# JohnLonginotto/uq

Hardware: AMD Instinct MI355X
Metric: FASTQ encode MB/s (150bp synthetic; bit-exact tables vs reference) (higher is better)
Workload: dtype u8

## Files before the change

uq_amd/csrc/pack.hip:

```cpp
#include "common.h"
#include "swar.h"
#include "lines.h"
#include "histo.h"

namespace {
constexpr int PK_THREADS = 256;

struct PackLut {
    int16_t dna_code[256];
    int16_t qual_code[256];
    int16_t n_qual[256];
};

struct PackGeom {
    uint32_t R;
    uint32_t Rs;
    uint32_t Cd, Cq;
    uint32_t G;
    uint32_t variable;
    uint32_t stage_bytes;
    uint32_t out_bytes;
    uint32_t magicG;
    uint32_t dna_max;
    uint32_t fill_d, fill_q;
// ... 27 lines not shown
    if constexpr ((4 * B) % 8 == 0) return i < B / 2 ? a1 >> (8 * i) : a0 >> (8 * (i - B / 2));
    else
#endif
    return (uint32_t)((((uint64_t)a0 << (4 * B)) | a1) >> (8 * i));
}

template <bool CLEAR = false>
__device__ __noinline__ void store_tile_any(uint8_t* gdst, uint8_t* lsrc, uint32_t nb, uint32_t tid) {
    const uint32_t mis = (uint32_t)(uintptr_t)gdst;
    if ((mis & 15) == 0) {
        const uint32_t nv = nb >> 4;
        for (uint32_t i = tid; i < nv; i += 256) { ((uint4*)gdst)[i] = ((const uint4*)lsrc)[i]; if (CLEAR) ((uint4*)lsrc)[i] = make_uint4(0, 0, 0, 0); }
        for (uint32_t i = (nv << 4) + tid; i < nb; i += 256) { gdst[i] = lsrc[i]; if (CLEAR) lsrc[i] = 0; }
    } else if ((mis & 7) == 0) {
        const uint32_t nv = nb >> 3;
        for (uint32_t i = tid; i < nv; i += 256) { ((uint2*)gdst)[i] = ((const uint2*)lsrc)[i]; if (CLEAR) ((uint2*)lsrc)[i] = make_uint2(0, 0); }
        for (uint32_t i = (nv << 3) + tid; i < nb; i += 256) { gdst[i] = lsrc[i]; if (CLEAR) lsrc[i] = 0; }
    } else if ((mis & 3) == 0) {
        const uint32_t nv = nb >> 2;
        for (uint32_t i = tid; i < nv; i += 256) { ((uint32_t*)gdst)[i] = ((const uint32_t*)lsrc)[i]; if (CLEAR) ((uint32_t*)lsrc)[i] = 0; }
        for (uint32_t i = (nv << 2) + tid; i < nb; i += 256) { gdst[i] = lsrc[i]; if (CLEAR) lsrc[i] = 0; }
    } else {
        for (uint32_t i = tid; i < nb; i += 256) { gdst[i] = lsrc[i]; if (CLEAR) lsrc[i] = 0; }
    }
}
template <bool CLEAR = false>
__device__ __forceinline__ void store_tile(uint8_t* gdst, uint8_t* lsrc, uint32_t nb, uint32_t tid) {
    if ((((uint32_t)(uintptr_t)gdst) & 15u) == 0 && (nb & 15u) == 0) {
#pragma unroll 1
        for (uint32_t i = tid; i < (nb >> 4); i += 256) { ((uint4*)gdst)[i] = ((const uint4*)lsrc)[i]; if (CLEAR) ((uint4*)lsrc)[i] = make_uint4(0, 0, 0, 0); }
    } else store_tile_any<CLEAR>(gdst, lsrc, nb, tid);
}

struct QnLds {
    uint8_t line1[256 + 16];
    uint8_t inset[256];
    uint8_t seps[32];
    uint32_t vmin[UQ_QF_MAXC], vmax[UQ_QF_MAXC];
    uint32_t flags, on, plen, slen, nsep, l1len;
    uint32_t sepset;
    uint32_t seps_lo, seps_hi;
    uint32_t pow10[10];
};

__device__ __forceinline__ uint32_t eq_bytes(uint32_t w, uint32_t c4) {
    const uint32_t x = w ^ c4;
    return ~((((x & 0x7F7F7F7Fu) + 0x7F7F7F7Fu) | x)) & 0x80808080u;
}
__device__ __forceinline__ uint32_t nondigit_bytes(uint32_t w) {
    const uint32_t lo7 = w & 0x7F7F7F7Fu;
    return (~(lo7 + 0x50505050u) | (lo7 + 0x46464646u) | w) & 0x80808080u;
}
__device__ __forceinline__ uint32_t low_bytes(uint32_t n) { return n >= 4 ? 0xFFFFFFFFu : ~(0xFFFFFFFFu << (8 * n)); }

__device__ __forceinline__ void lds_window12(const uint8_t* base, int32_t o, uint32_t& w0, uint32_t& w1, uint32_t& w2) {
    const uint32_t* p = (const uint32_t*)(base + (o & ~3));
    const uint32_t a = p[0], b = p[1], c = p[2], d = p[3];
    const uint32_t sh = (uint32_t)o & 3u;
    w0 = __builtin_amdgcn_alignbyte(b, a, sh);
    w1 = __builtin_amdgcn_alignbyte(c, b, sh);
    w2 = __builtin_amdgcn_alignbyte(d, c, sh);
}

__device__ __forceinline__ void qname_tile(const uint8_t* stage, const uint32_t* meta, uint32_t q, QnLds* s, uint32_t* __restrict__ vals, uint64_t pitch,
                                           uint64_t row) {
    const uint32_t qs = meta[4 * q], ql = meta[4 * q + 1] - qs - 1;
    const uint32_t plen = s->plen, slen = s->slen, nsep = s->nsep, l1len = s->l1len;
// ... 47 lines not shown
        }
        if (bad) f |= 16u;
        const unsigned long long want = (unsigned long long)s->seps_lo | ((unsigned long long)s->seps_hi << 32);
        if (found != nsep || eseq != want) f |= 1u;
        uint32_t start = plen;
        for (uint32_t c = 0; c <= nsep && c < UQ_QF_MAXC; ++c) {
            uint32_t stop = c == nsep ? end : (uint32_t)(epos >> (8 * c)) & 0xFFu;
            if (stop < start || stop > end) stop = start;
            const uint32_t nd = stop - start;
            uint32_t w0, w1, w2;
            lds_window12(stage, (int32_t)(qs + stop) - 12, w0, w1, w2);
            const uint32_t keep = nd > 9 ? 9u : nd;
            const uint32_t k2 = low_bytes(keep >= 4 ? 0u : 4u - keep), k1 = keep <= 4 ? 0xFFFFFFFFu : (keep >= 8 ? 0u : low_bytes(8u - keep)),
                           k0 = keep <= 8 ? 0xFFFFFFFFu : low_bytes(12u - keep);
            const uint32_t d0 = w0 & 0x0F0F0F0Fu & ~k0, d1 = w1 & 0x0F0F0F0Fu & ~k1, d2 = w2 & 0x0F0F0F0Fu & ~k2;
            uint32_t mag = d0 >> 24;
            mag = mag * 10 + (d1 & 0xFFu); mag = mag * 10 + ((d1 >> 8) & 0xFFu); mag = mag * 10 + ((d1 >> 16) & 0xFFu); mag = mag * 10 + (d1 >> 24);
            mag = mag * 10 + (d2 & 0xFFu); mag = mag * 10 + ((d2 >> 8) & 0xFFu); mag = mag * 10 + ((d2 >> 16) & 0xFFu); mag = mag * 10 + (d2 >> 24);
            if (nd > 9) f |= 4u;
            else if (nd == 0 || (nd > 1 && mag < s->pow10[nd - 1])) f |= 16u;
            vals[c * pitch + row] = mag;
            if (mag < s->vmin[c]) atomicMin(&s->vmin[c], mag);
            if (mag > s->vmax[c]) atomicMax(&s->vmax[c], mag);
            start = stop + 1;
        }
        if (ql < l1len && !differs && !(f & 32u)) f |= 128u;
        if (ql < l1len && s->line1[l1len - ql] == s->line1[0]) f |= 128u;
    }
    if (f) atomicOr(&s->flags, f);
}

constexpr int PK_NV = 5;
constexpr int PK_NV_STATS = 4;
#ifdef PK_ONE_COPY
constexpr int pks_copies(int bd, bool four_wg) { return bd == 3 ? 4 : 1; }
#else
constexpr int pks_copies(int bd, bool four_wg) { return bd == 2 && four_wg ? 8 : 4; }
#endif
constexpr uint32_t pks_bins(int bd) { return bd == 3 ? 512u : 256u; }
constexpr uint32_t pks_words(int bd, bool four_wg) { return pks_bins(bd) * pks_copies(bd, four_wg) + 128; }

struct TileRec { uint64_t start; uint32_t T, A, B, pad; };
struct PackLists {
    CensusView cv;
    const uint32_t* over;
};

__global__ __launch_bounds__(256) void tile_origin_kernel(CensusView cv, const unsigned long long* __restrict__ d_async, const uint32_t* __restrict__ over, uint64_t first,
                                                          uint64_t n, uint64_t R, uint64_t entries, TileRec* __restrict__ rec, unsigned long long* __restrict__ bad) {
    const uint64_t tt = (uint64_t)blockIdx.x * 256 + threadIdx.x;
    if (tt == 0) *bad = UQ_NONE;
    if (tt >= entries) return;
    uint64_t nlines = 4 * (first + n);
    if (d_async) {
        nlines = d_async[0];
        const uint64_t have = nlines / 4;
        if (have < n) n = have;
        if (d_async[1] || *over) n = 0;
    }
    uint64_t r = tt * R;
    if (r > n) r = n;
    uint32_t T, kk;
    cv_locate(cv, (int64_t)(4 * (first + r)) - 1, T, kk);
    bool ok;
    TileRec out;
    out.start = n ? cv_line_start(cv, nlines, T, kk, 0, ok) : 0;
    uint32_t c[3];
#pragma unroll
    for (uint32_t k = 0; k < 3; ++k) {
        const uint64_t t = (uint64_t)T + k;
        c[k] = t < cv.nb ? (uint32_t)((t + 1 < cv.nb ? (uint64_t)cv.offs[t + 1] : nlines) - cv.offs[t]) : 0u;
        if (c[k] > CV_LIST_CAP) c[k] = CV_LIST_CAP;
    }
    out.T = T; out.A = kk | (c[0] << 16); out.B = c[1] | (c[2] << 16); out.pad = 0;
    rec[tt] = out;
}

template <int BD, int BQ, bool NTRICK, bool FAST, bool STATS, bool QN, bool LISTS = false, bool VAR = false>
__global__ __launch_bounds__(PK_THREADS, (STATS && (NTRICK || QN)) ? 4 : 5) void pack_tile_kernel(const uint8_t* __restrict__ buf,
                                                               const uint64_t* __restrict__ ls, uint64_t first,
                                                               uint64_t n, PackLut lut, PackGeom g,
                                                               uint8_t* __restrict__ dna, uint8_t* __restrict__ qual,
                                                               unsigned long long* __restrict__ bad,
                                                               uq_stats* __restrict__ st, const unsigned long long* __restrict__ d_async,
                                                               uq_qname_fused* __restrict__ qf, uint32_t* __restrict__ qvals, uint64_t qpitch, PackLists pl,
                                                               const TileRec* __restrict__ trec) {
    constexpr int NV = STATS ? PK_NV_STATS : PK_NV;
    extern __shared__ __align__(16) uint8_t smem[];
    uint8_t* stage = smem + 16;
    uint8_t* out_d = stage + g.stage_bytes;
    uint32_t* meta = (uint32_t*)(out_d + g.out_bytes);
    int16_t* l_dna = (int16_t*)(meta + 4 * g.R + 4);
    int16_t* l_qual = l_dna + 256;
    int16_t* l_nq = l_qual + 256;

    const uint32_t tid = threadIdx.x;
    l_dna[tid] = lut.dna_code[tid];
    l_qual[tid] = lut.qual_code[tid];
    if (NTRICK) l_nq[tid] = lut.n_qual[tid];
    RecordAcc acc;
    bool incomplete = false;
    constexpr bool FOUR_WG = STATS && (NTRICK || QN);
    constexpr int PKS_COPIES = pks_copies(BD, FOUR_WG);
    __shared__ uint32_t cnt_tab[STATS ? pks_words(BD, FOUR_WG) : 1];
    uint32_t fill_pairs = 0, n_pairs = 0;
    constexpr uint32_t PKS_BINS = pks_bins(BD), PKS_WORDS = pks_words(BD, FOUR_WG);
    if (STATS) for (uint32_t i = tid; i < PKS_WORDS; i += PK_THREADS) cnt_tab[i] = 0;
    if (VAR) for (uint32_t i = tid; i < (g.out_bytes >> 4); i += PK_THREADS) ((uint4*)out_d)[i] = make_uint4(0, 0, 0, 0);
    QnLds* qn = (QnLds*)(l_nq + 256);
    bool qn_on = false;
    if (STATS && QN) qn_on = qf->ok != 0;
    if (STATS && QN) {
        qn->line1[tid] = qf->line1[tid]; qn->inset[tid] = qf->inset[tid];
        if (tid < 16) qn->line1[256 + tid] = 0;
        if (tid < 32) qn->seps[tid] = qf->seps[tid];
        if (tid < UQ_QF_MAXC) { qn->vmin[tid] = 0xFFFFFFFFu; qn->vmax[tid] = 0; }
        if (tid == 0) {
            qn->flags = 0; qn->plen = qf->plen; qn->slen = qf->slen; qn->nsep = qf->nsep; qn->l1len = qf->l1len;
            uint32_t set = 0x01010101u * qf->seps[0], nset = 1, lo = 0, hi = 0;
            for (uint32_t k = 0; k < qf->nsep && k < 8; ++k) {
                const uint32_t c = qf->seps[k];
                if (k < 4) lo |= c << (8 * k); else hi |= c << (8 * (k - 4));
                bool seen = false;
                for (uint32_t m = 0; m < nset; ++m) seen = seen || ((set >> (8 * m)) & 0xFFu) == c;
                if (!seen && nset < 4) { set = (set & ~(0xFFu << (8 * nset))) | (c << (8 * nset)); ++nset; }
            }
            qn->sepset = set; qn->seps_lo = lo; qn->seps_hi = hi;
            uint32_t pw = 1;
            for (uint32_t k = 0; k < 10; ++k) { qn->pow10[k] = pw; pw *= 10; }
        }
    }
    uint64_t nl_total = 4 * (first + n);
    constexpr bool lists = STATS && LISTS;
    if (d_async) {
        nl_total = d_async[0];
        const uint64_t have = d_async[0] / 4;
        if (have > n) incomplete = true; else n = have;
        if (d_async[1] || (lists && *pl.over)) { incomplete = true; n = 0; }
    }

    const uint64_t R = g.R;
    const uint64_t ntiles = (n + R - 1) / R;
    const uint64_t S = gridDim.x;
    struct Bounds { uint64_t g0, g1; uint32_t pT, pA, pB; };
    struct Regs { uint4 v[NV]; uint64_t m0; uint64_t g0; uint32_t skew, nvec, Rt, mrel, mraw; bool ok; };
    struct RawBounds { uint32_t lo, hi; };
    auto load_raw = [&](uint64_t tt) {
        RawBounds x{0u, 0u};
        if (tt < ntiles) {
            const uint32_t ln = lane_id();
            if constexpr (lists) {
                x.lo = ((const uint32_t*)(trec + tt))[ln < 8u ? ln : 0u];
            } else {
                const uint32_t Rn = (uint32_t)((n - tt * R) < R ? (n - tt * R) : R);
                const uint64_t v = ls[4 * (first + tt * R) + (ln == 1u ? 4 * Rn : 0u)];
                x.lo = (uint32_t)v; x.hi = (uint32_t)(v >> 32);
            }
        }
        return x;
    };
    auto bounds_of = [&](uint64_t tt, const RawBounds& x) {
        auto lane = [](uint32_t v, int k) { return (uint32_t)__builtin_amdgcn_readlane((int)v, k); };
        Bounds b{0, 0, 0, 0, 0};
        if (tt < ntiles) {
            if constexpr (lists) {
                b.g0 = (uint64_t)lane(x.lo, 0) | ((uint64_t)lane(x.lo, 1) << 32);
                b.pT = lane(x.lo, 2); b.pA = lane(x.lo, 3); b.pB = lane(x.lo, 4);
                b.g1 = (uint64_t)lane(x.lo, 6) | ((uint64_t)lane(x.lo, 7) << 32);
            } else {
                b.g0 = (uint64_t)lane(x.lo, 0) | ((uint64_t)lane(x.hi, 0) << 32);
                b.g1 = (uint64_t)lane(x.lo, 1) | ((uint64_t)lane(x.hi, 1) << 32);
            }
        }
        return b;
    };
    auto load_bounds = [&](uint64_t tt) {
        Bounds b{0, 0, 0, 0, 0};
        if (tt < ntiles) {
            const uint32_t Rn = (uint32_t)((n - tt * R) < R ? (n - tt * R) : R);
            if constexpr (lists) {
                const TileRec r0 = trec[tt];
                b.g0 = r0.start; b.pT = r0.T; b.pA = r0.A; b.pB = r0.B; b.g1 = trec[tt + 1].start;
            }
            else { b.g0 = ls[4 * (first + tt * R)]; b.g1 = ls[4 * (first + tt * R) + 4 * Rn]; }
        }
        return b;
    };
    auto tile_reads = [&](uint64_t tt) -> uint32_t { return tt < ntiles ? (uint32_t)((n - tt * R) < R ? (n - tt * R) : R) : 0u; };
    auto issue = [&](uint64_t rfirst, uint32_t cnt, Bounds b) {
        Regs x;
        x.ok = false; x.m0 = 0; x.g0 = b.g0; x.skew = 0; x.nvec = 0; x.Rt = 0; x.mrel = 0; x.mraw = 0;
#pragma unroll
        for (int u = 0; u < NV; ++u) x.v[u] = make_uint4(0, 0, 0, 0);
        if (cnt == 0) return x;
        x.Rt = cnt;
        const uint64_t a0 = ((uint64_t)(uintptr_t)buf + b.g0) & ~uint64_t(15);
        x.skew = (uint32_t)(((uint64_t)(uintptr_t)buf + b.g0) - a0);
        const uint64_t span = b.g1 - b.g0 + x.skew;
        x.nvec = (uint32_t)((span + 15) >> 4);
        x.ok = span + 32 <= g.stage_bytes && x.nvec <= (uint32_t)(NV * PK_THREADS);
        if constexpr (lists) {
            const uint32_t kk = b.pA & 0xFFFFu, avail = (b.pA >> 16) + (b.pB & 0xFFFFu) + (b.pB >> 16);
            if (kk + 4 * cnt > avail) x.ok = false;
        }
        if (!x.ok) return x;
        const uint4* src = (const uint4*)(buf + ((int64_t)b.g0 - (int64_t)x.skew));
#pragma unroll
        for (int u = 0; u < NV; ++u) { const uint32_t i = u * PK_THREADS + tid; if (i < x.nvec) x.v[u] = src[i]; }
        if (tid <= 4 * x.Rt) {
            if constexpr (lists) {
                uint32_t idx = (b.pA & 0xFFFFu) + tid, t = b.pT;
                const uint32_t c0 = b.pA >> 16, c1 = b.pB & 0xFFFFu;
                if (idx > c0) { idx -= c0; ++t; if (idx > c1) { idx -= c1; ++t; } }
                x.mrel = x.skew - (uint32_t)b.g0 + (idx == 0 ? 0u : (uint32_t)t * (uint32_t)CV_TILE - pl.cv.mis + 1u);
                x.mraw = idx == 0 ? 0u : (uint32_t)pl.cv.list[(uint64_t)t * CV_LIST_CAP + (idx - 1)];
            } else x.m0 = ls[4 * (first + rfirst) + tid];
        }
        return x;
    };

    uint32_t rr, pp;
    fast_divmod(tid, g.P, g.magicP, rr, pp);
    uint32_t badr = 0xFFFFFFFFu;
    uint64_t bad_tile = UQ_NONE;
    auto do_tile = [&](const uint64_t r0, const Regs& cur, auto&& between) {
        const uint32_t Rt = cur.Rt;
        uint8_t* out_q = out_d + ((Rt * g.Cd + 15) & ~15u);
        if (cur.ok) {
            if (tid <= 4 * Rt) meta[tid] = lists ? cur.mrel + cur.mraw : (uint32_t)(cur.m0 - cur.g0) + cur.skew;
#pragma unroll
            for (int u = 0; u < NV; ++u) { const uint32_t i = u * PK_THREADS + tid; if (i < cur.nvec) ((uint4*)stage)[i] = cur.v[u]; }
        } else {
            if (tid == 0) bad_tile = bad_tile < r0 ? bad_tile : r0;
            incomplete = true;
            if (STATS && QN && qn_on && tid == 0) atomicOr(&qf->flags, 256u);
        }
        __syncthreads();
        const bool ok = cur.ok;
        between();
#ifndef PK_ABL_NOQN
        if (STATS && QN && qn_on && ok && tid >= PK_THREADS - 64 && tid - (PK_THREADS - 64) < Rt)
            qname_tile(stage, meta, tid - (PK_THREADS - 64), qn, qvals, qpitch, r0 + (tid - (PK_THREADS - 64)));
#endif
        if (ok) {
            auto pack_group = [&](const uint32_t r, const uint32_t L, const int32_t wd, const uint32_t shd, const int32_t wq, const uint32_t shq, uint8_t* orow_d,
                                  uint8_t* orow_q, const uint32_t gg) {
                const int32_t j0 = (int32_t)L - 8 * (int32_t)gg - 8;
                uint32_t ad0 = 0, ad1 = 0, aq0 = 0, aq1 = 0;
                if (j0 > -8) {
                uint32_t b_lo, b_hi, q_lo, q_hi;
                lds_window8_at(stage, wd, shd, b_lo, b_hi);
                lds_window8_at(stage, wq, shq, q_lo, q_hi);
                if (j0 < 0) {
                    uint32_t mlo, mhi;
                    window_masks((uint32_t)(-j0), mlo, mhi);
                    b_lo = bfi(mlo, b_lo, g.fill_d); b_hi = bfi(mhi, b_hi, g.fill_d);
                    q_lo = bfi(mlo, q_lo, g.fill_q); q_hi = bfi(mhi, q_hi, g.fill_q);
                }
                bool generic = !FAST;
                if (FAST) {
                    uint32_t c0, c1, e0, e1;
                    if constexpr (BD == 2) {
                        c0 = acgt_codes(b_lo); c1 = acgt_codes(b_hi);
                        e0 = acgt_chars(c0) ^ b_lo; e1 = acgt_chars(c1) ^ b_hi;
                    } else {
                        c0 = __builtin_amdgcn_perm(g.i2c_hi, g.i2c_lo, (b_lo >> g.h_shift) & 0x07070707u);
                        c1 = __builtin_amdgcn_perm(g.i2c_hi, g.i2c_lo, (b_hi >> g.h_shift) & 0x07070707u);
                        e0 = __builtin_amdgcn_perm(g.c2c_hi, g.c2c_lo, c0) ^ b_lo; e1 = __builtin_amdgcn_perm(g.c2c_hi, g.c2c_lo, c1) ^ b_hi;
                    }
                    uint32_t u0 = q_lo + g.q_addlo, u1 = q_hi + g.q_addlo;
                    uint32_t bq0 = (q_lo | (q_lo + g.q_addhi) | ~u0) & 0x80808080u;
                    uint32_t bq1 = (q_hi | (q_hi + g.q_addhi) | ~u1) & 0x80808080u;
                    uint32_t x0 = u0 & 0x7F7F7F7Fu, x1 = u1 & 0x7F7F7F7Fu;
                    if (e0 | e1) {
                        if (NTRICK && !((q_lo | q_hi) & 0x80808080u)) {
// ... 34 lines not shown
                                    atomicAdd((uint32_t*)(hb + b0 * (4 * PKS_COPIES)), 1u);
                                    atomicAdd((uint32_t*)(hb + b1 * (4 * PKS_COPIES)), 1u);
                                }
                            }
                            if (j0 < 0) fill_pairs += (uint32_t)(-j0);
                            if (NTRICK && (e0 | e1)) {
                                const uint32_t m0 = nonzero_bytes(e0), m1 = nonzero_bytes(e1);
                                const uint32_t ne0 = nonzero_bytes(q_lo ^ g.n_qchar), ne1 = nonzero_bytes(q_hi ^ g.n_qchar);
                                n_pairs += (uint32_t)__popc(m0 & 0x01010101u) + (uint32_t)__popc(m1 & 0x01010101u);
                                if ((m0 & ne0) | (m1 & ne1)) incomplete = true;
                            }
                        }
                    }
                }
                if (generic) {
                    const uint32_t cbw[2] = {b_lo, b_hi};
                    const uint32_t cqw[2] = {q_lo, q_hi};
                    uint32_t ad[2] = {0, 0}, aq[2] = {0, 0};
                    int32_t orall = 0;
#pragma unroll
                    for (int k = 0; k < 8; ++k) {
                        const uint32_t cb = (cbw[k >> 2] >> (8 * (k & 3))) & 255u;
                        const uint32_t cc = (cqw[k >> 2] >> (8 * (k & 3))) & 255u;
                        int32_t dc = l_dna[cb];
                        int32_t qc = l_qual[cc];
                        if (NTRICK) {
                            if (dc < 0) { dc = 0; qc = l_nq[cb]; }
                        }
                        orall |= dc | qc;
                        ad[k >> 2] = (ad[k >> 2] << BD) | (uint32_t)dc;
                        aq[k >> 2] = (aq[k >> 2] << BQ) | (uint32_t)qc;
                    }
                    if (orall < 0) {
                        badr = badr < (uint32_t)(r0 + r) ? badr : (uint32_t)(r0 + r);
                        ad[0] = ad[1] = aq[0] = aq[1] = 0;
                    }
                    ad0 = ad[0]; ad1 = ad[1]; aq0 = aq[0]; aq1 = aq[1];
                }
                }
                if (g.variable) {
                    const int32_t i = (int32_t)L - 8 * (int32_t)gg;
                    if (i >= 0 && i < 4) { ad1 |= 1u << (BD * i); aq1 |= 1u << (BQ * i); }
                    else if (i >= 4 && i < 8) { ad0 |= 1u << (BD * (i - 4)); aq0 |= 1u << (BQ * (i - 4)); }
                }
                uint8_t* od = orow_d - BD * gg;
                uint8_t* oq = orow_q - BQ * gg;
#ifdef PK_ABL_NOSTORE
                if ((ad0 ^ aq0) == 0x12345678u && (ad1 ^ aq1) == 0x9ABCDEF0u) od[0] = 1;
                else if (false)
#endif
                if (gg + 1 < g.G) {
#pragma unroll
                    for (int i = 0; i < BD; ++i) od[-i] = (uint8_t)group_byte<BD>(ad0, ad1, i);
#pragma unroll
                    for (int i = 0; i < BQ; ++i) oq[-i] = (uint8_t)group_byte<BQ>(aq0, aq1, i);
                } else {
                    const uint32_t nd = g.Cd - BD * gg, nq = g.Cq - BQ * gg;
#pragma unroll
                    for (int i = 0; i < BD; ++i)
                        if ((uint32_t)i < nd) od[-i] = (uint8_t)group_byte<BD>(ad0, ad1, i);
#pragma unroll
                    for (int i = 0; i < BQ; ++i)
                        if ((uint32_t)i < nq) oq[-i] = (uint8_t)group_byte<BQ>(aq0, aq1, i);
                }
            };
            if (rr < Rt) {
                const uint32_t r = rr;
                const uint32_t so = meta[4 * r + 1];
                uint32_t L = meta[4 * r + 2] - so - 1;
                const uint32_t qo = meta[4 * r + 3];
                if (STATS) {
                    const uint32_t Lq = meta[4 * r + 4] - qo - 1;
#ifndef PK_ABL_NOREC
                    if (pp == 0) acc.record(r0 + r, stage[meta[4 * r + 2]] == '+', L, Lq, meta[4 * r + 4] - meta[4 * r]);
#endif
                    if (L > g.dna_max || Lq != L) incomplete = true;
                }
                if (L > g.dna_max || meta[4 * r + 4] - qo - 1 != L) { badr = badr < (uint32_t)(r0 + r) ? badr : (uint32_t)(r0 + r); L = 0; }
                uint8_t* orow_d = out_d + r * g.Cd + (g.Cd - 1);
                uint8_t* orow_q = out_q + r * g.Cq + (g.Cq - 1);
                const uint32_t gend = VAR ? (((L + 8) >> 3) < g.G ? ((L + 8) >> 3) : g.G) : g.G;
#ifndef PK_ABL_NOGROUP
                int32_t wd = (int32_t)(so + L) - 8 * (int32_t)pp - 8, wq = (int32_t)(qo + L) - 8 * (int32_t)pp - 8;
                const uint32_t shd = (uint32_t)wd & 3u, shq = (uint32_t)wq & 3u;
                wd &= ~3; wq &= ~3;
                const int32_t wstep = 8 * (int32_t)g.P;
                for (uint32_t gg = pp; gg < gend; gg += g.P, wd -= wstep, wq -= wstep) pack_group(r, L, wd, shd, wq, shq, orow_d, orow_q, gg);
#endif
            }
        }
        __syncthreads();
#ifndef PK_NO_EARLY_WAIT
        __builtin_amdgcn_s_waitcnt(0x0F70);
#endif
        if (ok) {
            if constexpr (STATS && (NTRICK || QN)) {
                store_tile<VAR>(dna + r0 * g.Cd, out_d, Rt * g.Cd, tid);
                store_tile<VAR>(qual + r0 * g.Cq, out_q, Rt * g.Cq, tid);
            } else {
                store_tile_any<VAR>(dna + r0 * g.Cd, out_d, Rt * g.Cd, tid);
                store_tile_any<VAR>(qual + r0 * g.Cq, out_q, Rt * g.Cq, tid);
            }
        }
    };

    uint64_t t = blockIdx.x;
    constexpr bool VBOUNDS = STATS && (NTRICK || QN);
    using NextBounds = std::conditional_t<VBOUNDS, RawBounds, Bounds>;
    auto fetch_next = [&](uint64_t tt) -> NextBounds { if constexpr (VBOUNDS) return load_raw(tt); else return load_bounds(tt); };
    auto next_bounds = [&](uint64_t tt, const NextBounds& x) -> Bounds { if constexpr (VBOUNDS) return bounds_of(tt, x); else return x; };
    NextBounds b_next = fetch_next(t + S);
    Regs cur = issue(t * R, tile_reads(t), load_bounds(t));
#ifndef PK_NO_EARLY_WAIT
    __builtin_amdgcn_s_waitcnt(0x0F70);
#endif
    for (; t < ntiles; t += S) {
        NextBounds b_nn{};
        if constexpr (!VBOUNDS) b_nn = fetch_next(t + 2 * S);
        if (cur.ok) {
            const Regs now = cur;
            do_tile(t * R, now, [&] {
                cur = issue((t + S) * R, tile_reads(t + S), next_bounds(t + S, b_next));
                if constexpr (VBOUNDS) b_next = fetch_next(t + 2 * S); else b_next = b_nn;
            });
        } else {
            const uint32_t Rt = cur.Rt;
            for (uint32_t sub = 0; sub < Rt; sub += g.Rs) {
                const uint32_t cnt = Rt - sub < g.Rs ? Rt - sub : g.Rs;
                const uint64_t rf = t * R + sub;
                Bounds sb{0, 0, 0, 0, 0};
                if constexpr (lists) {
                    uint32_t T, kk; bool found;
                    cv_locate(pl.cv, (int64_t)(4 * (first + rf)) - 1, T, kk);
                    sb.g0 = cv_line_start(pl.cv, nl_total, T, kk, 0, found); sb.g1 = cv_line_start(pl.cv, nl_total, T, kk, 4 * cnt, found);
                    uint32_t c[3];
#pragma unroll
                    for (uint32_t k = 0; k < 3; ++k) {
                        const uint64_t tq = (uint64_t)T + k;
                        c[k] = tq < pl.cv.nb ? (uint32_t)((tq + 1 < pl.cv.nb ? (uint64_t)pl.cv.offs[tq + 1] : nl_total) - pl.cv.offs[tq]) : 0u;
                        if (c[k] > CV_LIST_CAP) c[k] = CV_LIST_CAP;
                    }
                    sb.pT = T; sb.pA = kk | (c[0] << 16); sb.pB = c[1] | (c[2] << 16);
                } else { sb.g0 = ls[4 * (first + rf)]; sb.g1 = ls[4 * (first + rf) + 4 * cnt]; }
                const Regs piece = issue(rf, cnt, sb);
                do_tile(rf, piece, [] {});
                __syncthreads();
            }
            cur = issue((t + S) * R, tile_reads(t + S), next_bounds(t + S, b_next));
            if constexpr (VBOUNDS) b_next = fetch_next(t + 2 * S); else b_next = b_nn;
#ifndef PK_NO_EARLY_WAIT
            __builtin_amdgcn_s_waitcnt(0x0F70);
#endif
        }
    }
    if (badr != 0xFFFFFFFFu) atomicMin(bad, (unsigned long long)badr);
    if (bad_tile != UQ_NONE) atomicMin(bad, (unsigned long long)bad_tile);
    if (STATS) {
        if (fill_pairs) atomicSub(&cnt_tab[lane_id() & (PKS_COPIES - 1)], fill_pairs);
        if (NTRICK && n_pairs) {
            atomicSub(&cnt_tab[((g.n_code & 0xFFu) * PKS_COPIES) + (lane_id() & (PKS_COPIES - 1))], n_pairs);
            atomicAdd(&cnt_tab[PKS_BINS * PKS_COPIES], n_pairs);
        }
        __syncthreads();
        const uint32_t qmin = 0x80u - (g.q_addlo & 0xFFu);
        for (uint32_t bin = tid; bin < PKS_BINS; bin += PK_THREADS) {
            uint32_t v = 0;
#pragma unroll
            for (int c = 0; c < PKS_COPIES; ++c) v += cnt_tab[bin * PKS_COPIES + c];
            const uint32_t code = bin >> 6;
            const uint32_t base = BD == 2 ? (0x54474341u >> (8 * code)) & 0xFFu
                                          : ((code < 4 ? g.c2c_lo >> (8 * code) : g.c2c_hi >> (8 * (code - 4))) & 0xFFu);
            if (v) atomicAdd((unsigned long long*)&st->counts[base * 256 + qmin + (bin & 63u)], (unsigned long long)v);
        }
        if (NTRICK && tid == 0) {
            const uint32_t v = cnt_tab[PKS_BINS * PKS_COPIES];
            if (v) atomicAdd((unsigned long long*)&st->counts[(g.n_char & 0xFFu) * 256 + (g.n_qchar & 0xFFu)], (unsigned long long)v);
        }
        acc.flush(st, first);
        if (incomplete) st->reserved = 1;
        if (QN) {
            if (qn_on && tid < UQ_QF_MAXC && qn->vmin[tid] <= qn->vmax[tid]) { atomicMin(&qf->vmin[tid], qn->vmin[tid]); atomicMax(&qf->vmax[tid], qn->vmax[tid]); }
            if (qn_on && tid == 0 && qn->flags) atomicOr(&qf->flags, qn->flags);
            if (blockIdx.x == 0 && tid == 0) qf->nreads = n;
        }
    }
}

__global__ __launch_bounds__(256) void pack_carry_kernel(const uint8_t* __restrict__ buf, const uint64_t* __restrict__ ls,
                                                         uint64_t first, uint64_t n, PackLut lut, uint32_t bd, uint32_t bq,
                                                         uint32_t Cd, uint32_t Cq, uint32_t variable,
                                                         uint8_t* __restrict__ dna, uint8_t* __restrict__ qual,
                                                         unsigned long long* __restrict__ bad) {
    __shared__ int16_t l_dna[256], l_qual[256], l_nq[256];
    l_dna[threadIdx.x] = lut.dna_code[threadIdx.x];
    l_qual[threadIdx.x] = lut.qual_code[threadIdx.x];
    l_nq[threadIdx.x] = lut.n_qual[threadIdx.x];
    __syncthreads();
    const uint64_t r = (uint64_t)blockIdx.x * blockDim.x + threadIdx.x;
    if (r >= n) return;
    const uint64_t* p = ls + 4 * (first + r);
    const uint64_t s = p[1], q = p[3];
    const uint32_t L = (uint32_t)(p[2] - s - 1);
    uint8_t* drow = dna + r * Cd;
    uint8_t* qrow = qual + r * Cq;
    uint32_t td = 0, tq = 0, bdn = 0, bqn = 0;
    int32_t pd = (int32_t)Cd - 1, pq = (int32_t)Cq - 1;
    for (uint32_t t = 0; t < L; ++t) {
        uint32_t cb = buf[s + L - 1 - t], cc = buf[q + L - 1 - t];
        int dc = l_dna[cb], qc = l_qual[cc];
        if (dc < 0) { dc = 0; qc = l_nq[cb]; }
        if (qc < 0) { atomicMin(bad, (unsigned long long)r); qc = 0; }
        td += (uint32_t)dc << bdn; tq += (uint32_t)qc << bqn;
        bdn += bd; bqn += bq;
        while (bdn > 8) { bdn -= 8; if (pd >= 0) drow[pd] = (uint8_t)td; td >>= 8; --pd; }
        while (bqn > 8) { bqn -= 8; if (pq >= 0) qrow[pq] = (uint8_t)tq; tq >>= 8; --pq; }
    }
// ... 21 lines not shown
    if (var && lists) {
        if (qn) return bd == 3 ? pick_stats_kernel_q<3, true, true, true>(bq, ntrick) : pick_stats_kernel_q<2, true, true, true>(bq, ntrick);
        return bd == 3 ? pick_stats_kernel_q<3, false, true, true>(bq, ntrick) : pick_stats_kernel_q<2, false, true, true>(bq, ntrick);
    }
    if (qn && lists) return bd == 3 ? pick_stats_kernel_q<3, true, true>(bq, ntrick) : pick_stats_kernel_q<2, true, true>(bq, ntrick);
    if (lists) return bd == 3 ? pick_stats_kernel_q<3, false, true>(bq, ntrick) : pick_stats_kernel_q<2, false, true>(bq, ntrick);
    if (bd == 3) return qn ? pick_stats_kernel_q<3, true>(bq, ntrick) : pick_stats_kernel_q<3, false>(bq, ntrick);
    return qn ? pick_stats_kernel_q<2, true>(bq, ntrick) : pick_stats_kernel_q<2, false>(bq, ntrick);
}

template <int BD>
PackKernel pick_bq(int bq, bool ntrick, bool fast) {
    switch (bq) {
        case 1: return pick_nt<BD, 1>(ntrick, fast); case 2: return pick_nt<BD, 2>(ntrick, fast); case 3: return pick_nt<BD, 3>(ntrick, fast);
        case 4: return pick_nt<BD, 4>(ntrick, fast); case 5: return pick_nt<BD, 5>(ntrick, fast); case 6: return pick_nt<BD, 6>(ntrick, fast);
        case 7: return pick_nt<BD, 7>(ntrick, fast); default: return pick_nt<BD, 8>(ntrick, fast);
    }
}

PackKernel pick_kernel(int bd, int bq, bool ntrick, bool fast) {
    switch (bd) {
        case 1: return pick_bq<1>(bq, ntrick, fast); case 2: return pick_bq<2>(bq, ntrick, fast); case 3: return pick_bq<3>(bq, ntrick, fast);
        case 4: return pick_bq<4>(bq, ntrick, fast); case 5: return pick_bq<5>(bq, ntrick, fast); case 6: return pick_bq<6>(bq, ntrick, fast);
        case 7: return pick_bq<7>(bq, ntrick, fast); default: return pick_bq<8>(bq, ntrick, fast);
    }
}
}

static int pack_impl(uq_ctx* ctx, const uint8_t* d_buf, const uint64_t* d_line_start, uint64_t first_read,
                     uint64_t nreads, const uq_pack_params* hp, uint8_t* d_dna, uint8_t* d_qual, uint64_t* d_bad,
                     uq_stats* d_stats, int* h_fused, const unsigned long long* d_async = nullptr, uq_qname_fused* d_q = nullptr,
                     uint32_t* d_vals = nullptr, uint64_t vals_pitch = 0) {
    const bool use_lists = d_line_start == nullptr && d_async != nullptr && d_stats != nullptr;
    UQ_REQUIRE(ctx && d_buf && (d_line_start || use_lists) && hp && d_dna && d_qual && d_bad, "uq_pack: null argument");
    UQ_REQUIRE(!use_lists || (ctx->async_buf == d_buf && ctx->async_nbytes > 0), "uq_pack_stats_async: no line index given and no census of this buffer queued in front");
    if (h_fused) *h_fused = 0;
    ctx->pk_stats = ctx->pk_q = nullptr;
    if (d_stats && ctx->stats_sent == (const void*)d_stats) ctx->stats_sent = nullptr;
    UQ_REQUIRE(hp->bits_per_base >= 1 && hp->bits_per_base <= 8 && hp->bits_per_quality >= 1 && hp->bits_per_quality <= 8,
               "uq_pack: bits per symbol must be 1..8");
    const uint32_t bd = hp->bits_per_base, bq = hp->bits_per_quality;
    const uint32_t Cd = hp->dna_bytes_per_row, Cq = hp->quality_bytes_per_row;
    const uint32_t Lv = hp->dna_max + (hp->variable ? 1 : 0);
    UQ_REQUIRE(Cd == (bd * Lv + 7) / 8 && Cq == (bq * Lv + 7) / 8,
               "uq_pack: row bytes (%u, %u) do not match ceil(bits * (dna_max + variable) / 8)", Cd, Cq);
    struct BadGuard {
        uint64_t* p; hipStream_t s; bool armed;
        ~BadGuard() { if (armed) (void)hipMemsetAsync(p, 0xFF, 8, s); }
    } bad_guard{d_bad, ctx->stream, use_lists && nreads != 0};
    if (!bad_guard.armed) UQ_CHECK_HIP(hipMemsetAsync(d_bad, 0xFF, 8, ctx->stream));
    if (nreads == 0) return 0;

    PackLut lut;
    int max_d = 0, max_q = 0;
    bool ntrick = false;
    int fill_d = -1, fill_q = -1;
    for (int i = 0; i < 256; ++i) {
        lut.dna_code[i] = hp->dna_code[i];
        lut.qual_code[i] = hp->qual_code[i];
        lut.n_qual[i] = (int16_t)(hp->n_qual[i] > 32767 ? 32767 : hp->n_qual[i]);
        if (hp->dna_code[i] > max_d) max_d = hp->dna_code[i];
        if (hp->qual_code[i] > max_q) max_q = hp->qual_code[i];
        if (hp->dna_code[i] < 0 && hp->n_qual[i] >= 0) { ntrick = true; if (hp->n_qual[i] > max_q) max_q = hp->n_qual[i]; }
        if (hp->dna_code[i] == 0 && fill_d < 0) fill_d = i;
        if (hp->qual_code[i] == 0 && fill_q < 0) fill_q = i;
    }
// ... 11 lines not shown
                                                           hp->variable ? 1u : 0u, d_dna, d_qual, (unsigned long long*)d_bad);
        UQ_LAUNCH_CHECK();
        return 0;
    }

    PackGeom g;
    g.Cd = Cd; g.Cq = Cq; g.variable = hp->variable ? 1 : 0;
    g.G = (Lv + 7) / 8;
    g.dna_max = (uint32_t)hp->dna_max;
    g.magicG = magic_u32(g.G);
    g.fill_d = 0x01010101u * (uint32_t)fill_d;
    g.fill_q = 0x01010101u * (uint32_t)fill_q;
    uint32_t Rs = (stage_cap - 64) / rec;
    if (Rs > (PK_THREADS - 1) / 4) Rs = (PK_THREADS - 1) / 4;
    if (Rs == 0) Rs = 1;
    uint32_t R = Rs;
    const uint32_t avg = (uint32_t)hp->avg_record_bytes;
    if (avg >= 4 && avg < rec) {
        R = (stage_cap - 64) / (avg + avg * 15 / 100 + 1);
        if (R > (PK_THREADS - 1) / 4) R = (PK_THREADS - 1) / 4;
        if (R < Rs) R = Rs;
    }
    {
        const uint32_t out_cap = stage_cap * 3 / 4, fit = out_cap / (Cd + Cq);
        if (R > fit) R = fit > Rs ? fit : Rs;
    }
    if (R >= 4) {
        const uint32_t r16 = R & ~15u, r8 = R & ~7u, r4 = R & ~3u;
        if (r16 * 100 >= R * 85) R = r16; else if (r8 * 100 >= R * 85) R = r8; else R = r4;
    }
    if (R == 0) R = 1;
    if (Rs > R) Rs = R;
    g.R = R; g.Rs = Rs;
    g.stage_bytes = stage_cap + 32;
    g.out_bytes = (((R * Cd + 15) & ~15u) + R * Cq + 15) & ~15u;
    uint32_t P = (d_q ? PK_THREADS - 64 : PK_THREADS) / R;
    if (P > g.G) P = g.G;
    if (P < 1) P = 1;
    g.P = P; g.magicP = magic_u32(P);
    bool fast = bd == 2 && hp->dna_code['A'] == 0 && hp->dna_code['C'] == 1 && hp->dna_code['G'] == 2 && hp->dna_code['T'] == 3;
    int nbases = 0, nq = 0, qmin = 256, qmaxc = -1, ntrick_bases = 0, nchar = 0;
    for (int i = 0; i < 256; ++i) {
        if (hp->dna_code[i] >= 0) ++nbases;
        if (hp->qual_code[i] >= 0) { ++nq; if (i < qmin) qmin = i; if (i > qmaxc) qmaxc = i; }
        if (hp->dna_code[i] < 0 && hp->n_qual[i] >= 0) { ++ntrick_bases; nchar = i; }
    }
    g.h_shift = g.i2c_lo = g.i2c_hi = g.c2c_lo = g.c2c_hi = 0;
    bool fast3 = false;
    if (bd == 3 && nbases >= 1 && nbases <= 8) {
        for (uint32_t sh = 0; sh <= 4 && !fast3; ++sh) {
            uint8_t i2c[8], c2c[8]; bool used[8] = {false, false, false, false, false, false, false, false};
            memset(i2c, 0, 8); memset(c2c, 0, 8);
            bool ok = true;
            for (int ch = 1; ch < 128 && ok; ++ch) {
                const int code = hp->dna_code[ch];
                if (code < 0) continue;
                const uint32_t idx = ((uint32_t)ch >> sh) & 7u;
                if (used[idx] || code > 7) ok = false;
                else { used[idx] = true; i2c[idx] = (uint8_t)code; c2c[code] = (uint8_t)ch; }
            }
            for (int ch = 128; ch < 256 && ok; ++ch) if (hp->dna_code[ch] >= 0) ok = false;
            if (ok) {
                fast3 = true; g.h_shift = sh;
                memcpy(&g.i2c_lo, i2c, 4); memcpy(&g.i2c_hi, i2c + 4, 4); memcpy(&g.c2c_lo, c2c, 4); memcpy(&g.c2c_hi, c2c + 4, 4);
            }
        }
    }
    fast = ((fast && nbases == 4) || fast3) && nq >= 1 && qmaxc - qmin + 1 == nq && qmaxc < 128 && ntrick_bases <= 1 &&
           (ntrick_bases == 0 || (hp->n_qual[nchar] < 128 && nchar < 128));
    if (fast)
        for (int i = qmin; i <= qmaxc; ++i) fast = fast && hp->qual_code[i] == i - qmin;
    g.q_addlo = g.q_addhi = g.n_char = g.n_code = g.n_qchar = 0;
    if (fast) {
        g.q_addlo = 0x01010101u * (uint32_t)(0x80 - qmin);
        g.q_addhi = 0x01010101u * (uint32_t)(0x80 - qmin - nq);
        if (ntrick_bases == 1) {
            g.n_char = 0x01010101u * (uint32_t)nchar; g.n_code = 0x01010101u * (uint32_t)hp->n_qual[nchar];
            g.n_qchar = 0x01010101u * (uint32_t)(qmin + hp->n_qual[nchar]);
        }
    }
    if (d_stats && ((ntrick_bases == 1 && hp->n_qual[nchar] >= nq) ||
                    !fast || (bd != 2 && bd != 3) || bq > 6)) {
        return 0;
    }
    const bool var_deal = d_stats && use_lists && hp->variable;
    const size_t lds_static = d_stats ? pks_words((int)bd, ntrick || d_q != nullptr) * 4 : 4;
    const size_t lds = 16 + (size_t)g.stage_bytes + g.out_bytes + (4 * R + 4) * 4 + 3 * 512 + (d_stats ? sizeof(QnLds) : 0);
    UQ_REQUIRE(lds + lds_static <= 160 * 1024, "uq_pack: tile needs %zu bytes of LDS", lds + lds_static);
    const uint64_t tiles = (nreads + R - 1) / R;
    PackKernel k = d_stats ? pick_stats_kernel((int)bd, (int)bq, ntrick, d_q != nullptr, use_lists, var_deal) : pick_kernel((int)bd, (int)bq, ntrick, fast);
    if (lds > 48 * 1024) UQ_CHECK_HIP(hipFuncSetAttribute((const void*)k, hipFuncAttributeMaxDynamicSharedMemorySize, (int)lds));
    uint32_t per_cu = (uint32_t)((160 * 1024) / (lds + lds_static));
    {
        int cached_regs = 0;
        for (int i = 0; i < ctx->kreg_n; ++i) if (ctx->kreg_key[i] == (const void*)k) cached_regs = ctx->kreg_val[i];
        if (cached_regs == 0) {
            hipFuncAttributes fa;
            UQ_CHECK_HIP(hipFuncGetAttributes(&fa, (const void*)k));
            cached_regs = fa.numRegs > 0 ? fa.numRegs : 128;
            const int slot = ctx->kreg_n < 8 ? ctx->kreg_n++ : 7;
            ctx->kreg_key[slot] = (const void*)k; ctx->kreg_val[slot] = cached_regs;
        }
        const uint32_t alloc = ((uint32_t)(cached_regs > 0 ? cached_regs : 128) + 7) & ~7u;
        uint32_t waves_per_simd = 512 / alloc; if (waves_per_simd > 8) waves_per_simd = 8; if (waves_per_simd < 1) waves_per_simd = 1;
        const uint32_t waves_per_wg = PK_THREADS / 64;
        const uint32_t by_regs = 4 * waves_per_simd / waves_per_wg;
        if (by_regs >= 1 && by_regs < per_cu) per_cu = by_regs;
    }
    if (per_cu > 6) per_cu = 6;
    if (per_cu < 1) per_cu = 1;
    const uint64_t blocks = tiles < (uint64_t)UQ_NUM_CU * per_cu ? tiles : (uint64_t)UQ_NUM_CU * per_cu;
    PackLists pl;
    memset(&pl, 0, sizeof(pl));
    const TileRec* trec = nullptr;
    if (use_lists) {
        const uint32_t mis = (uint32_t)((uintptr_t)d_buf & 15);
        pl.cv.list = ctx->idx_bitmap; pl.cv.offs = ctx->idx_partials; pl.cv.mis = mis;
        pl.cv.nb = (((ctx->async_nbytes + mis + 15) / 16) * 16 + CV_TILE - 1) / CV_TILE;
        const uint64_t entries = tiles + 1;
// ... 54 lines not shown
```

Measured before the change: 1.474 million.

## Cut scalar register pressure in pack kernel via 32-bit indices and LDS-parked args

Switches the tile and read indices in the pack kernel from 64-bit to 32-bit, capping a call at 2^31 reads, so address arithmetic needs fewer registers. In the four-workgroup stats variants, rarely used kernel arguments (pointers, first, nl_total, Rs, census nb) are parked in LDS and reloaded only where needed. LDS is also reordered so the stage size is a compile-time constant and the lookup tables and metadata come before the variable-size output buffer. The aim is to lower SGPR/VGPR pressure and spills to help occupancy. The cost is a small extra LDS footprint, an added barrier on the sub-tile path, and the new read-count limit.

```diff
diff --git a/uq_amd/csrc/pack.hip b/uq_amd/csrc/pack.hip
--- a/uq_amd/csrc/pack.hip
+++ b/uq_amd/csrc/pack.hip
@@ -83,7 +83,7 @@
     } else store_tile_any<CLEAR>(gdst, lsrc, nb, tid);
 }
 
-struct QnLds {
+struct alignas(16) QnLds {
     uint8_t line1[256 + 16];
     uint8_t inset[256];
     uint8_t seps[32];
@@ -197,6 +197,7 @@
 
 constexpr int PK_NV = 5;
 constexpr int PK_NV_STATS = 4;
+constexpr uint32_t pk_stage_bytes(bool stats) { return (uint32_t)(stats ? PK_NV_STATS : PK_NV) * PK_THREADS * 16 + 32; }
 #ifdef PK_ONE_COPY
 constexpr int pks_copies(int bd, bool four_wg) { return bd == 3 ? 4 : 1; }
 #else
@@ -206,6 +207,7 @@
 constexpr uint32_t pks_words(int bd, bool four_wg) { return pks_bins(bd) * pks_copies(bd, four_wg) + 128; }
 
 struct TileRec { uint64_t start; uint32_t T, A, B, pad; };
+struct PkParked { unsigned long long* bad; uq_stats* st; uq_qname_fused* qf; uint64_t first, nb, nl_total; uint32_t Rs, pad; };
 struct PackLists {
     CensusView cv;
     const uint32_t* over;
@@ -252,12 +254,14 @@
                                                                const TileRec* __restrict__ trec) {
     constexpr int NV = STATS ? PK_NV_STATS : PK_NV;
     extern __shared__ __align__(16) uint8_t smem[];
+    constexpr uint32_t STAGE_BYTES = pk_stage_bytes(STATS);
     uint8_t* stage = smem + 16;
-    uint8_t* out_d = stage + g.stage_bytes;
-    uint32_t* meta = (uint32_t*)(out_d + g.out_bytes);
-    int16_t* l_dna = (int16_t*)(meta + 4 * g.R + 4);
+    int16_t* l_dna = (int16_t*)(stage + STAGE_BYTES);
     int16_t* l_qual = l_dna + 256;
     int16_t* l_nq = l_qual + 256;
+    QnLds* qn = (QnLds*)(l_nq + 256);
+    uint32_t* meta = (uint32_t*)((uint8_t*)qn + (STATS ? sizeof(QnLds) : 0));
+    uint8_t* out_d = (uint8_t*)(meta + 4 * g.R + 4);
 
     const uint32_t tid = threadIdx.x;
     l_dna[tid] = lut.dna_code[tid];
@@ -272,7 +276,6 @@
     constexpr uint32_t PKS_BINS = pks_bins(BD), PKS_WORDS = pks_words(BD, FOUR_WG);
     if (STATS) for (uint32_t i = tid; i < PKS_WORDS; i += PK_THREADS) cnt_tab[i] = 0;
     if (VAR) for (uint32_t i = tid; i < (g.out_bytes >> 4); i += PK_THREADS) ((uint4*)out_d)[i] = make_uint4(0, 0, 0, 0);
-    QnLds* qn = (QnLds*)(l_nq + 256);
     bool qn_on = false;
     if (STATS && QN) qn_on = qf->ok != 0;
     if (STATS && QN) {
@@ -295,36 +298,51 @@
             for (uint32_t k = 0; k < 10; ++k) { qn->pow10[k] = pw; pw *= 10; }
         }
     }
+    uint32_t nr = (uint32_t)n;
+#if defined(__HIP_DEVICE_COMPILE__)
+    asm("" : "+s"(nr));
+#endif
     uint64_t nl_total = 4 * (first + n);
     constexpr bool lists = STATS && LISTS;
     if (d_async) {
         nl_total = d_async[0];
         const uint64_t have = d_async[0] / 4;
-        if (have > n) incomplete = true; else n = have;
-        if (d_async[1] || (lists && *pl.over)) { incomplete = true; n = 0; }
-    }
-
-    const uint64_t R = g.R;
-    const uint64_t ntiles = (n + R - 1) / R;
-    const uint64_t S = gridDim.x;
+        if (have > nr) incomplete = true; else nr = (uint32_t)have;
+        if (d_async[1] || (lists && *pl.over)) { incomplete = true; nr = 0; }
+    }
+
+    __shared__ PkParked parked;
+    if constexpr (FOUR_WG) {
+        if (tid == 0) { parked.bad = bad; parked.st = st; parked.qf = qf; parked.first = first; parked.nb = pl.cv.nb; parked.nl_total = nl_total; parked.Rs = g.Rs; }
+    }
+    auto p_bad = [&] { if constexpr (FOUR_WG) return parked.bad; else return bad; };
+    auto p_st = [&] { if constexpr (FOUR_WG) return parked.st; else return st; };
+    auto p_qf = [&] { if constexpr (FOUR_WG) return parked.qf; else return qf; };
+    auto p_first = [&] { if constexpr (FOUR_WG) return parked.first; else return first; };
+    auto p_nl_total = [&] { if constexpr (FOUR_WG) return parked.nl_total; else return nl_total; };
+    auto p_Rs = [&] { if constexpr (FOUR_WG) return parked.Rs; else return g.Rs; };
+    auto p_cv = [&] { CensusView v = pl.cv; if constexpr (FOUR_WG) v.nb = parked.nb; return v; };
+    const uint32_t R = g.R;
+    const uint32_t ntiles = (nr + R - 1) / R;
+    const uint32_t S = gridDim.x;
     struct Bounds { uint64_t g0, g1; uint32_t pT, pA, pB; };
     struct Regs { uint4 v[NV]; uint64_t m0; uint64_t g0; uint32_t skew, nvec, Rt, mrel, mraw; bool ok; };
     struct RawBounds { uint32_t lo, hi; };
-    auto load_raw = [&](uint64_t tt) {
+    auto load_raw = [&](uint32_t tt) {
         RawBounds x{0u, 0u};
         if (tt < ntiles) {
             const uint32_t ln = lane_id();
             if constexpr (lists) {
                 x.lo = ((const uint32_t*)(trec + tt))[ln < 8u ? ln : 0u];
             } else {
-                const uint32_t Rn = (uint32_t)((n - tt * R) < R ? (n - tt * R) : R);
-                const uint64_t v = ls[4 * (first + tt * R) + (ln == 1u ? 4 * Rn : 0u)];
+                const uint32_t Rn = (nr - tt * R) < R ? (nr - tt * R) : R;
+                const uint64_t v = ls[4 * (first + (uint64_t)tt * R) + (ln == 1u ? 4 * Rn : 0u)];
                 x.lo = (uint32_t)v; x.hi = (uint32_t)(v >> 32);
             }
         }
         return x;
     };
-    auto bounds_of = [&](uint64_t tt, const RawBounds& x) {
+    auto bounds_of = [&](uint32_t tt, const RawBounds& x) {
         auto lane = [](uint32_t v, int k) { return (uint32_t)__builtin_amdgcn_readlane((int)v, k); };
         Bounds b{0, 0, 0, 0, 0};
         if (tt < ntiles) {
@@ -339,20 +357,20 @@
         }
         return b;
     };
-    auto load_bounds = [&](uint64_t tt) {
+    auto load_bounds = [&](uint32_t tt) {
         Bounds b{0, 0, 0, 0, 0};
         if (tt < ntiles) {
-            const uint32_t Rn = (uint32_t)((n - tt * R) < R ? (n - tt * R) : R);
+            const uint32_t Rn = (nr - tt * R) < R ? (nr - tt * R) : R;
             if constexpr (lists) {
                 const TileRec r0 = trec[tt];
                 b.g0 = r0.start; b.pT = r0.T; b.pA = r0.A; b.pB = r0.B; b.g1 = trec[tt + 1].start;
             }
-            else { b.g0 = ls[4 * (first + tt * R)]; b.g1 = ls[4 * (first + tt * R) + 4 * Rn]; }
+            else { b.g0 = ls[4 * (first + (uint64_t)tt * R)]; b.g1 = ls[4 * (first + (uint64_t)tt * R) + 4 * Rn]; }
         }
         return b;
     };
-    auto tile_reads = [&](uint64_t tt) -> uint32_t { return tt < ntiles ? (uint32_t)((n - tt * R) < R ? (n - tt * R) : R) : 0u; };
-    auto issue = [&](uint64_t rfirst, uint32_t cnt, Bounds b) {
+    auto tile_reads = [&](uint32_t tt) -> uint32_t { return tt < ntiles ? ((nr - tt * R) < R ? (nr - tt * R) : R) : 0u; };
+    auto issue = [&](uint32_t rfirst, uint32_t cnt, Bounds b) {
         Regs x;
         x.ok = false; x.m0 = 0; x.g0 = b.g0; x.skew = 0; x.nvec = 0; x.Rt = 0; x.mrel = 0; x.mraw = 0;
 #pragma unroll
@@ -363,7 +381,7 @@
         x.skew = (uint32_t)(((uint64_t)(uintptr_t)buf + b.g0) - a0);
         const uint64_t span = b.g1 - b.g0 + x.skew;
         x.nvec = (uint32_t)((span + 15) >> 4);
-        x.ok = span + 32 <= g.stage_bytes && x.nvec <= (uint32_t)(NV * PK_THREADS);
+        x.ok = span + 32 <= STAGE_BYTES && x.nvec <= (uint32_t)(NV * PK_THREADS);
         if constexpr (lists) {
             const uint32_t kk = b.pA & 0xFFFFu, avail = (b.pA >> 16) + (b.pB & 0xFFFFu) + (b.pB >> 16);
             if (kk + 4 * cnt > avail) x.ok = false;
@@ -379,7 +397,7 @@
                 if (idx > c0) { idx -= c0; ++t; if (idx > c1) { idx -= c1; ++t; } }
                 x.mrel = x.skew - (uint32_t)b.g0 + (idx == 0 ? 0u : (uint32_t)t * (uint32_t)CV_TILE - pl.cv.mis + 1u);
                 x.mraw = idx == 0 ? 0u : (uint32_t)pl.cv.list[(uint64_t)t * CV_LIST_CAP + (idx - 1)];
-            } else x.m0 = ls[4 * (first + rfirst) + tid];
+            } else x.m0 = ls[4 * (first + (uint64_t)rfirst) + tid];
         }
         return x;
     };
@@ -387,8 +405,8 @@
     uint32_t rr, pp;
     fast_divmod(tid, g.P, g.magicP, rr, pp);
     uint32_t badr = 0xFFFFFFFFu;
-    uint64_t bad_tile = UQ_NONE;
-    auto do_tile = [&](const uint64_t r0, const Regs& cur, auto&& between) {
+    uint32_t bad_tile = 0xFFFFFFFFu;
+    auto do_tile = [&](const uint32_t r0, const Regs& cur, auto&& between) {
         const uint32_t Rt = cur.Rt;
         uint8_t* out_q = out_d + ((Rt * g.Cd + 15) & ~15u);
         if (cur.ok) {
@@ -398,14 +416,14 @@
         } else {
             if (tid == 0) bad_tile = bad_tile < r0 ? bad_tile : r0;
             incomplete = true;
-            if (STATS && QN && qn_on && tid == 0) atomicOr(&qf->flags, 256u);
+            if (STATS && QN && qn_on && tid == 0) atomicOr(&p_qf()->flags, 256u);
         }
         __syncthreads();
         const bool ok = cur.ok;
         between();
 #ifndef PK_ABL_NOQN
         if (STATS && QN && qn_on && ok && tid >= PK_THREADS - 64 && tid - (PK_THREADS - 64) < Rt)
-            qname_tile(stage, meta, tid - (PK_THREADS - 64), qn, qvals, qpitch, r0 + (tid - (PK_THREADS - 64)));
+            qname_tile(stage, meta, tid - (PK_THREADS - 64), qn, qvals, qpitch, (uint64_t)r0 + (tid - (PK_THREADS - 64)));
 #endif
         if (ok) {
             auto pack_group = [&](const uint32_t r, const uint32_t L, const int32_t wd, const uint32_t shd, const int32_t wq, const uint32_t shq, uint8_t* orow_d,
@@ -506,7 +524,7 @@
                         aq[k >> 2] = (aq[k >> 2] << BQ) | (uint32_t)qc;
                     }
                     if (orall < 0) {
-                        badr = badr < (uint32_t)(r0 + r) ? badr : (uint32_t)(r0 + r);
+                        badr = badr < r0 + r ? badr : r0 + r;
                         ad[0] = ad[1] = aq[0] = aq[1] = 0;
                     }
                     ad0 = ad[0]; ad1 = ad[1]; aq0 = aq[0]; aq1 = aq[1];
@@ -550,7 +568,7 @@
 #endif
                     if (L > g.dna_max || Lq != L) incomplete = true;
                 }
-                if (L > g.dna_max || meta[4 * r + 4] - qo - 1 != L) { badr = badr < (uint32_t)(r0 + r) ? badr : (uint32_t)(r0 + r); L = 0; }
+                if (L > g.dna_max || meta[4 * r + 4] - qo - 1 != L) { badr = badr < r0 + r ? badr : r0 + r; L = 0; }
                 uint8_t* orow_d = out_d + r * g.Cd + (g.Cd - 1);
                 uint8_t* orow_q = out_q + r * g.Cq + (g.Cq - 1);
                 const uint32_t gend = VAR ? (((L + 8) >> 3) < g.G ? ((L + 8) >> 3) : g.G) : g.G;
@@ -569,20 +587,20 @@
 #endif
         if (ok) {
             if constexpr (STATS && (NTRICK || QN)) {
-                store_tile<VAR>(dna + r0 * g.Cd, out_d, Rt * g.Cd, tid);
-                store_tile<VAR>(qual + r0 * g.Cq, out_q, Rt * g.Cq, tid);
+                store_tile<VAR>(dna + (uint64_t)r0 * g.Cd, out_d, Rt * g.Cd, tid);
+                store_tile<VAR>(qual + (uint64_t)r0 * g.Cq, out_q, Rt * g.Cq, tid);
             } else {
-                store_tile_any<VAR>(dna + r0 * g.Cd, out_d, Rt * g.Cd, tid);
-                store_tile_any<VAR>(qual + r0 * g.Cq, out_q, Rt * g.Cq, tid);
+                store_tile_any<VAR>(dna + (uint64_t)r0 * g.Cd, out_d, Rt * g.Cd, tid);
+                store_tile_any<VAR>(qual + (uint64_t)r0 * g.Cq, out_q, Rt * g.Cq, tid);
             }
         }
     };
 
-    uint64_t t = blockIdx.x;
+    uint32_t t = blockIdx.x;
     constexpr bool VBOUNDS = STATS && (NTRICK || QN);
     using NextBounds = std::conditional_t<VBOUNDS, RawBounds, Bounds>;
-    auto fetch_next = [&](uint64_t tt) -> NextBounds { if constexpr (VBOUNDS) return load_raw(tt); else return load_bounds(tt); };
-    auto next_bounds = [&](uint64_t tt, const NextBounds& x) -> Bounds { if constexpr (VBOUNDS) return bounds_of(tt, x); else return x; };
+    auto fetch_next = [&](uint32_t tt) -> NextBounds { if constexpr (VBOUNDS) return load_raw(tt); else return load_bounds(tt); };
+    auto next_bounds = [&](uint32_t tt, const NextBounds& x) -> Bounds { if constexpr (VBOUNDS) return bounds_of(tt, x); else return x; };
     NextBounds b_next = fetch_next(t + S);
     Regs cur = issue(t * R, tile_reads(t), load_bounds(t));
 #ifndef PK_NO_EARLY_WAIT
@@ -599,23 +617,27 @@
             });
         } else {
             const uint32_t Rt = cur.Rt;
-            for (uint32_t sub = 0; sub < Rt; sub += g.Rs) {
-                const uint32_t cnt = Rt - sub < g.Rs ? Rt - sub : g.Rs;
-                const uint64_t rf = t * R + sub;
+            __syncthreads();
+            const uint32_t Rs = p_Rs();
+            for (uint32_t sub = 0; sub < Rt; sub += Rs) {
+                const uint32_t cnt = Rt - sub < Rs ? Rt - sub : Rs;
+                const uint32_t rf = t * R + sub;
                 Bounds sb{0, 0, 0, 0, 0};
                 if constexpr (lists) {
                     uint32_t T, kk; bool found;
-                    cv_locate(pl.cv, (int64_t)(4 * (first + rf)) - 1, T, kk);
-                    sb.g0 = cv_line_start(pl.cv, nl_total, T, kk, 0, found); sb.g1 = cv_line_start(pl.cv, nl_total, T, kk, 4 * cnt, found);
+                    const CensusView cv = p_cv();
+                    const uint64_t nl_total = p_nl_total();
+                    cv_locate(cv, (int64_t)(4 * (p_first() + rf)) - 1, T, kk);
+                    sb.g0 = cv_line_start(cv, nl_total, T, kk, 0, found); sb.g1 = cv_line_start(cv, nl_total, T, kk, 4 * cnt, found);
                     uint32_t c[3];
 #pragma unroll
                     for (uint32_t k = 0; k < 3; ++k) {
                         const uint64_t tq = (uint64_t)T + k;
-                        c[k] = tq < pl.cv.nb ? (uint32_t)((tq + 1 < pl.cv.nb ? (uint64_t)pl.cv.offs[tq + 1] : nl_total) - pl.cv.offs[tq]) : 0u;
+                        c[k] = tq < cv.nb ? (uint32_t)((tq + 1 < cv.nb ? (uint64_t)cv.offs[tq + 1] : nl_total) - cv.offs[tq]) : 0u;
                         if (c[k] > CV_LIST_CAP) c[k] = CV_LIST_CAP;
                     }
                     sb.pT = T; sb.pA = kk | (c[0] << 16); sb.pB = c[1] | (c[2] << 16);
-                } else { sb.g0 = ls[4 * (first + rf)]; sb.g1 = ls[4 * (first + rf) + 4 * cnt]; }
+                } else { sb.g0 = ls[4 * (first + (uint64_t)rf)]; sb.g1 = ls[4 * (first + (uint64_t)rf) + 4 * cnt]; }
                 const Regs piece = issue(rf, cnt, sb);
                 do_tile(rf, piece, [] {});
                 __syncthreads();
@@ -627,8 +649,8 @@
 #endif
         }
     }
-    if (badr != 0xFFFFFFFFu) atomicMin(bad, (unsigned long long)badr);
-    if (bad_tile != UQ_NONE) atomicMin(bad, (unsigned long long)bad_tile);
+    if (badr != 0xFFFFFFFFu) atomicMin(p_bad(), (unsigned long long)badr);
+    if (bad_tile != 0xFFFFFFFFu) atomicMin(p_bad(), (unsigned long long)bad_tile);
     if (STATS) {
         if (fill_pairs) atomicSub(&cnt_tab[lane_id() & (PKS_COPIES - 1)], fill_pairs);
         if (NTRICK && n_pairs) {
@@ -637,6 +659,8 @@
         }
         __syncthreads();
         const uint32_t qmin = 0x80u - (g.q_addlo & 0xFFu);
+        uq_stats* const st = p_st();
+        uq_qname_fused* const qf = p_qf();
         for (uint32_t bin = tid; bin < PKS_BINS; bin += PK_THREADS) {
             uint32_t v = 0;
 #pragma unroll
@@ -650,12 +674,12 @@
             const uint32_t v = cnt_tab[PKS_BINS * PKS_COPIES];
             if (v) atomicAdd((unsigned long long*)&st->counts[(g.n_char & 0xFFu) * 256 + (g.n_qchar & 0xFFu)], (unsigned long long)v);
         }
-        acc.flush(st, first);
+        acc.flush(st, p_first());
         if (incomplete) st->reserved = 1;
         if (QN) {
             if (qn_on && tid < UQ_QF_MAXC && qn->vmin[tid] <= qn->vmax[tid]) { atomicMin(&qf->vmin[tid], qn->vmin[tid]); atomicMax(&qf->vmax[tid], qn->vmax[tid]); }
             if (qn_on && tid == 0 && qn->flags) atomicOr(&qf->flags, qn->flags);
-            if (blockIdx.x == 0 && tid == 0) qf->nreads = n;
+            if (blockIdx.x == 0 && tid == 0) qf->nreads = nr;
         }
     }
 }
@@ -743,6 +767,7 @@
                      uq_stats* d_stats, int* h_fused, const unsigned long long* d_async = nullptr, uq_qname_fused* d_q = nullptr,
                      uint32_t* d_vals = nullptr, uint64_t vals_pitch = 0) {
     const bool use_lists = d_line_start == nullptr && d_async != nullptr && d_stats != nullptr;
+    UQ_REQUIRE(nreads <= (1ull << 31), "uq_pack: %llu reads in one call (at most 2^31)", (unsigned long long)nreads);
     UQ_REQUIRE(ctx && d_buf && (d_line_start || use_lists) && hp && d_dna && d_qual && d_bad, "uq_pack: null argument");
     UQ_REQUIRE(!use_lists || (ctx->async_buf == d_buf && ctx->async_nbytes > 0), "uq_pack_stats_async: no line index given and no census of this buffer queued in front");
     if (h_fused) *h_fused = 0;
@@ -820,7 +845,7 @@
     if (R == 0) R = 1;
     if (Rs > R) Rs = R;
     g.R = R; g.Rs = Rs;
-    g.stage_bytes = stage_cap + 32;
+    g.stage_bytes = pk_stage_bytes(d_stats != nullptr);
     g.out_bytes = (((R * Cd + 15) & ~15u) + R * Cq + 15) & ~15u;
     uint32_t P = (d_q ? PK_THREADS - 64 : PK_THREADS) / R;
     if (P > g.G) P = g.G;
@@ -872,7 +897,7 @@
         return 0;
     }
     const bool var_deal = d_stats && use_lists && hp->variable;
-    const size_t lds_static = d_stats ? pks_words((int)bd, ntrick || d_q != nullptr) * 4 : 4;
+    const size_t lds_static = d_stats ? pks_words((int)bd, ntrick || d_q != nullptr) * 4 + ((ntrick || d_q != nullptr) ? ((sizeof(PkParked) + 15) & ~size_t(15)) : 0) : 4;
     const size_t lds = 16 + (size_t)g.stage_bytes + g.out_bytes + (4 * R + 4) * 4 + 3 * 512 + (d_stats ? sizeof(QnLds) : 0);
     UQ_REQUIRE(lds + lds_static <= 160 * 1024, "uq_pack: tile needs %zu bytes of LDS", lds + lds_static);
     const uint64_t tiles = (nreads + R - 1) / R;
```

Measured after the change: 1.509 million (median of 6 runs). 1.02x the previous value.
